# germannp/yalla

Hardware: AMD Instinct MI355X
Metric: cell-updates/sec at 1M cells (Grid_solver) (higher is better)
Workload: dtype f32

## Files before the change

include/solvers.cuh:

```cuda
#pragma once

#include <hip/hip_runtime.h>
#include <hip/hip_ext.h>

#include <assert.h>
#include <math.h>
#include <stdio.h>
#include <stdlib.h>
#include <string.h>

#include <functional>
#include <mutex>
#include <type_traits>
#include <utility>
#include <vector>

#include "cudebug.cuh"
#include "dtypes.cuh"
#include "fold256.cuh"
#include "yalla_hip.h"

#ifndef YALLA_NO_THRUST
#include <thrust/execution_policy.h>
#include <thrust/fill.h>
// ... 1543 lines not shown
        return float3{f.src[0], f.src[1], f.src[2]};
    else if constexpr (S == Fix_src::partials)
        return fixed_velocity_from_partials<N_floats<Pt>::value>(f.src, f.arg, n);
    else
        return fix_from_total(f.src, N_floats<Pt>::value, f.arg);
}
template<typename Pt>
__device__ __forceinline__ Pt minus_fix(Pt dX, const float3 fix)
{
    dX.x -= fix.x;
    dX.y -= fix.y;
    dX.z -= fix.z;
    return dX;
}
template<typename Pt>
__device__ __forceinline__ Pt heun_row(const int i, const float dt, const float* __restrict__ d_fix, const float3 fix1,
    Pt* __restrict__ d_dX, const Pt* __restrict__ d_dX1, Pt* __restrict__ d_X, float3* __restrict__ d_old_v,
    const bool zero_dX)
{
    const Pt dX_raw = d_dX[i];
    if (zero_dX) d_dX[i] = ya::zero<Pt>();
    const Pt dX = minus_fix(dX_raw, float3{d_fix[0], d_fix[1], d_fix[2]});
    const Pt dX1 = minus_fix(d_dX1[i], fix1);
    Pt X = d_X[i];
    X += (dX + dX1) * 0.5 * dt;
    d_X[i] = X;
    d_old_v[i] = float3{(dX.x + dX1.x) * 0.5f, (dX.y + dX1.y) * 0.5f, (dX.z + dX1.z) * 0.5f};
    return X;
}
}


template<typename Pt, ya::Fix_src S>
__global__ __launch_bounds__(ya::UPDATE_BLOCK) void euler_step(const int n, const float dt, const ya::Fix_args fix_args,
    const Pt* __restrict__ d_dX, const Pt* __restrict__ d_X0, Pt* __restrict__ d_X1, const Pt* __restrict__ d_dX_sorted,
    ya::Entry<Pt>* __restrict__ d_sorted, const int n_active, Pt* __restrict__ d_zero, float* __restrict__ pred_partial,
    const ya::Guard_band band)
{
    const float3 fix = ya::resolve_fix<S, Pt>(fix_args, n);
    const int i = blockIdx.x * ya::UPDATE_BLOCK + threadIdx.x;
    if (i == 0 && fix_args.out) {
        fix_args.out[0] = fix.x;
        fix_args.out[1] = fix.y;
        fix_args.out[2] = fix.z;
    }
    float moved = 0.f;
    if (i < n) {
        if (d_X1) {
            const Pt X0 = d_X0[i];
            const Pt X1 = X0 + ya::minus_fix(d_dX[i], fix) * dt;
            d_X1[i] = X1;
            moved = fabsf(X1.z - X0.z) * band.weight(X0.z);
        }
        if (d_sorted) {
            ya::Entry<Pt> e = d_sorted[i];
            Pt dX = d_dX_sorted[i];
            if constexpr (S == ya::Fix_src::totals)
                if (e.id >= n_active) dX = d_dX[e.id];
            const float z0 = e.X.z;
            e.X = e.X + ya::minus_fix(dX, fix) * dt;
            d_sorted[i] = e;
            moved = fabsf(e.X.z - z0) * band.weight(z0);
        }
        if (d_zero) d_zero[i] = ya::zero<Pt>();
    }
    if constexpr (S == ya::Fix_src::totals)
        if (pred_partial) ya::block_max_to(moved, pred_partial);
}

template<typename Pt, ya::Fix_src S>
__global__ __launch_bounds__(ya::UPDATE_BLOCK) void heun_step(const int n, const float dt, const float* __restrict__ d_fix,
    const ya::Fix_args fix1_args, Pt* __restrict__ d_dX, const Pt* __restrict__ d_dX1, Pt* __restrict__ d_X,
    float3* __restrict__ d_old_v, const bool zero_dX, const float* __restrict__ z_selected,
    float* __restrict__ moved_partial, const ya::Guard_band band, float* __restrict__ votes_out)
{
    const float3 fix1 = ya::resolve_fix<S, Pt>(fix1_args, n);
    const int i = blockIdx.x * ya::UPDATE_BLOCK + threadIdx.x;
    float moved = 0.f;
    if (i < n) {
        const Pt X = ya::heun_row(i, dt, d_fix, fix1, d_dX, d_dX1, d_X, d_old_v, zero_dX);
        if (z_selected) moved = fabsf(X.z - z_selected[i]) * band.weight(z_selected[i]);
    }
    if constexpr (S == ya::Fix_src::totals) {
        if (votes_out && i == 0) {
            votes_out[0] = fix1_args.src[ya::N_floats<Pt>::value + 2];
            votes_out[1] = fix1_args.src[ya::N_floats<Pt>::value + 3];
        }
        if (moved_partial) ya::block_max_to(moved, moved_partial);
    }
}


namespace ya {
template<typename T>
__global__ __launch_bounds__(UPDATE_BLOCK) void permute_rows(const int n, const int* __restrict__ order,
    const T* __restrict__ src, T* __restrict__ dst)
{
    const int s = blockIdx.x * UPDATE_BLOCK + threadIdx.x;
    if (s < n) dst[s] = src[order[s]];
}
__global__ __launch_bounds__(UPDATE_BLOCK) void invert_order(const int n, const int* __restrict__ order,
    int* __restrict__ new_id)
{
// ... 31 lines not shown
        else
            h_X = (Pt*)calloc(n_max, sizeof(Pt));
    }
    ~Solution()
    {
        if (h_X_locked)
            (void)ya_host_free(h_X);
        else
            free(h_X);
        free(h_n);
    }
    Solution(const Solution&) = delete;

private:
    bool h_X_locked = false;

public:
    void copy_to_device()
    {
        assert(*h_n <= n_max);
        YA_CHECK(ya_memcpy_h2d(d_X, h_X, (size_t)n_max * sizeof(Pt)));
        YA_CHECK(ya_memcpy_h2d(d_n, h_n, sizeof(int)));
    }
    void copy_to_host()
    {
        YA_CHECK(ya_memcpy_d2h(h_X, d_X, (size_t)n_max * sizeof(Pt)));
        YA_CHECK(ya_memcpy_d2h(h_n, d_n, sizeof(int)));
        assert(*h_n <= n_max);
        Solver<Pt>::check_status();
    }
    int get_d_n() { return Solver<Pt>::get_d_n(); }
    template<Pairwise_interaction<Pt> pw_int>
    void take_step(float dt, Generic_forces<Pt> gen_forces = no_gen_forces<Pt>)
    {
        return Solver<Pt>::template take_step<pw_int, friction_w_neighbour<Pt>>(
            dt, gen_forces);
    }
    template<Pairwise_interaction<Pt> pw_int, Pairwise_friction<Pt> pw_friction>
    void take_step(float dt, Generic_forces<Pt> gen_forces = no_gen_forces<Pt>)
    {
        return Solver<Pt>::template take_step<pw_int, pw_friction>(dt, gen_forces);
    }
    template<Pairwise_interaction<Pt> pw_int, typename Gen2,
        typename = decltype(std::declval<Gen2&>()((const Pt*)nullptr, (Pt*)nullptr))>
    void take_step(float dt, Gen2 gen_forces)
    {
        take_step<pw_int>(dt, Generic_forces<Pt>{[gen_forces](const int, const Pt* d_X,
                                                     Pt* d_dX) mutable { gen_forces(d_X, d_dX); }});
    }
    template<Pairwise_interaction<Pt> pw_int, Pairwise_friction<Pt> pw_friction, typename Gen2,
        typename = decltype(std::declval<Gen2&>()((const Pt*)nullptr, (Pt*)nullptr))>
    void take_step(float dt, Gen2 gen_forces)
    {
        take_step<pw_int, pw_friction>(dt,
            Generic_forces<Pt>{[gen_forces](const int, const Pt* d_X, Pt* d_dX) mutable {
                gen_forces(d_X, d_dX);
// ... 84 lines not shown
    }

    template<typename... Arrays>
    void keep_in_cube_order(const int every, Arrays&... arrays)
    {
        keep_order_every = every;
        keep_order_wait = 0;
        if (every > 0)
            keep_order = [this, &arrays...]() { this->renumber(arrays...); };
        else
            keep_order = nullptr;
    }

    int graph_steps = 0;
    long graph_launches = 0;

protected:
#ifndef YA_GRAPH_MAX_CELLS
#define YA_GRAPH_MAX_CELLS 400000
#endif
    struct Step_key {
        const void* functors = nullptr;
        int n = -1;
        float dt = 0, cube_size = 0;
        typename Computer<Pt>::Step_variant variant{};
        int fix_mode = 0, fix_point = 0;
        bool fold = true;
        bool operator==(const Step_key& o) const
        {
            return functors == o.functors && n == o.n && dt == o.dt && cube_size == o.cube_size &&
// ... 234 lines not shown
        if (Computer<Pt>::use_sorted_pipeline()) {
            Computer<Pt>::begin_build(d_X, d_n, n_max, n_reader);
            YA_CHECK(ya_n_read_end(n_reader, &n));
            assert(n <= n_max);
        } else {
            n = get_d_n();
        }
        if (n <= 0) {
            Computer<Pt>::cancel_build();
            return;
        }

        heun_stages<pw_int, pw_friction>(n, dt, gen_forces);
        last_key = sorted_path ? key_of<pw_int, pw_friction>(n, dt) : Step_key{};
    }
};


const auto TILE_SIZE = 32;

template<typename Pt>
class Tile_computer {
public:
    Tile_computer(int n_max) {}
    ya::Profiler profiler;
    bool use_sorted_pipeline() const { return false; }
    int lanes_per_cell = 0;

protected:
    hipStream_t stream = nullptr;
    float step_cube_size() const { return 0; }
    using Step_variant = int;
    Step_variant step_variant() const { return 0; }
    template<Pairwise_interaction<Pt> pw_int, Pairwise_friction<Pt> pw_friction>
    bool ready_to_capture(int) const { return false; }
    void check_status() {}
    void begin_build(const Pt*, const int*, int, ya_n_reader*) {}
    void cancel_build() {}
    const int* cube_order(int, const Pt*) { return nullptr; }
    void ids_changed() {}
    const Pt* sorted_rhs() const { return nullptr; }
    ya::Entry<Pt>* sorted_cells() { return nullptr; }
    template<Pairwise_interaction<Pt> pw_int, Pairwise_friction<Pt> pw_friction>
    void pwints_from_sorted(int, Pt*, int, bool) {}
    template<Pairwise_interaction<Pt> pw_int, Pairwise_friction<Pt> pw_friction>
    void pwints(const int n, const Pt* __restrict__ d_X, const float3* __restrict__ d_old_v,
        Pt* d_dX, const bool has_gen, const int n_active, const bool keep_sorted)
    {
        assert(n_active == n);
        hipEvent_t start, stop;
        profiler.next(&start, &stop);
        int lanes = lanes_per_cell;
        if (lanes == 0) lanes = ya::stateless_pair<Pt, pw_int, pw_friction>() ? (n <= 4096 ? 64 : 16) : 1;
        if (lanes >= 64)
            hipExtLaunchKernelGGL((ya::tile_force_coop<Pt, pw_int, pw_friction, 64>), dim3((n + 3) / 4),
                dim3(256), 0, stream, start, stop, 0, n, d_X, d_old_v, d_dX, has_gen);
        else if (lanes > 1)
            hipExtLaunchKernelGGL((ya::tile_force_coop<Pt, pw_int, pw_friction, 16>), dim3((n + 15) / 16),
                dim3(256), 0, stream, start, stop, 0, n, d_X, d_old_v, d_dX, has_gen);
// ... 49 lines not shown
    template<typename Pt>
    void build_sorted_begin(const Pt* d_X, const int* d_n, const int n_bound, const float cube_size, ya_n_reader* reader)
    {
        YA_CHECK(ya_grid_build_sorted_begin_publish(handle, d_X, sizeof(Pt), d_n, n_bound, cube_size, reader, nullptr));
    }
    template<typename Pt>
    void build_sorted_finish(const int n, const Pt* d_X, const float3* d_old_v,
        ya::Entry<Pt>* d_sorted, float4* d_sorted_v)
    {
        YA_CHECK(ya_grid_build_sorted_finish(handle, d_X, sizeof(Pt), d_old_v, n, d_sorted,
            sizeof(ya::Entry<Pt>), d_sorted_v, nullptr));
    }
    template<typename Pt>
    void rebuild_sorted(const int n, const ya::Entry<Pt>* d_prev, const float4* d_prev_v,
        const float cube_size, ya::Entry<Pt>* d_sorted, float4* d_sorted_v,
        hipStream_t stream = nullptr)
    {
        YA_CHECK(ya_grid_rebuild_sorted(handle, d_prev, sizeof(ya::Entry<Pt>), sizeof(Pt),
            d_prev_v, n, cube_size, d_sorted, d_sorted_v, stream));
    }
    const int* offsets() const { return d_offs; }
    void forget_order() { YA_CHECK(ya_grid_forget_order(handle)); }
    void set_cube_range(const int cube_lo, const int cube_hi) { YA_CHECK(ya_grid_set_cube_range(handle, cube_lo, cube_hi)); }
    void check_status()
    {
        int bits = 0;
        YA_CHECK(ya_grid_status(handle, &bits, 1));
        if (bits & YA_STATUS_OUT_OF_RANGE) {
            fprintf(stderr,
                "yalla-hip: a cell left the cube range its z-slab promised the grid (Grid::set_cube_range): it "
                "moved more than a cube between two selections of the mirrored cells.\n");
            abort();
        }
        if (bits & YA_STATUS_SCAN_STALLED) {
// ... 48 lines not shown
                        (x - 1) + shift[y] * grid_size + shift[z] * grid_size * grid_size;
        YA_CHECK((int)hipMemcpyToSymbol(HIP_SYMBOL(d_nhood), h_nhood, sizeof(h_nhood)));
        YA_CHECK(ya_malloc((void**)&d_sorted, (size_t)n_max * sizeof(ya::Entry<Pt>)));
        YA_CHECK(ya_malloc((void**)&d_sorted_v, (size_t)n_max * sizeof(float4)));
        YA_CHECK(ya_malloc((void**)&d_resorted, (size_t)n_max * sizeof(ya::Entry<Pt>)));
        YA_CHECK(ya_malloc((void**)&d_resorted_v, (size_t)n_max * sizeof(float4)));
        YA_CHECK(ya_malloc((void**)&d_dX_sorted, (size_t)n_max * sizeof(Pt)));
    }
    ~Grid_computer()
    {
        ya_free(d_sorted);
        ya_free(d_sorted_v);
        ya_free(d_resorted);
        ya_free(d_resorted_v);
        ya_free(d_dX_sorted);
        for (int p = 0; p < 3; p++) ya_free(d_tail_exchange[p]), ya_free(d_tail_tickets[p]);
        if (interior_stream && interior_stream_owned) (void)hipStreamDestroy(interior_stream);
        if (grid_built) {
            (void)hipEventDestroy(grid_built);
            (void)hipEventDestroy(interior_done);
        }
    }
    Grid_computer(const Grid_computer&) = delete;
    int force_tail_tiles = -1;
    float* d_tail_exchange[3] = {nullptr, nullptr, nullptr};
    int* d_tail_tickets[3] = {nullptr, nullptr, nullptr};
    int tail_room[3] = {0, 0, 0};
    template<auto Kernel>
    static int resident_workgroups()
    {
// ... 256 lines not shown
            grid.build_sorted_finish(n, d_X, d_old_v, d_sorted, d_sorted_v);
        else
            grid.build_sorted(n, d_X, d_old_v, cube_size, d_sorted, d_sorted_v, stream);
        build_begun = false;
        forces<pw_int, pw_friction>(n, d_sorted, d_sorted_v, d_dX, has_gen, n_active,
            keep_sorted ? d_dX_sorted : nullptr);
    }
    const Pt* sorted_rhs() const { return d_dX_sorted; }
    ya::Entry<Pt>* sorted_cells() { return d_sorted; }
    template<Pairwise_interaction<Pt> pw_int, Pairwise_friction<Pt> pw_friction>
    void pwints_from_sorted(const int n, Pt* d_dX, const int n_active, const bool has_gen)
    {
        grid.rebuild_sorted(n, d_sorted, d_sorted_v, cube_size, d_resorted, d_resorted_v, stream);
        forces<pw_int, pw_friction>(n, d_resorted, d_resorted_v, d_dX, has_gen, n_active, nullptr);
    }
};

template<typename Pt>
using Grid_solver = Heun_solver<Pt, Grid_computer>;


template<typename Pt>
class Gabriel_computer : public Grid_computer<Pt> {
public:
    float gabriel_coefficient;
    Gabriel_computer(
        int n_max, int grid_size = 50, float cube_size = 1, float gabriel_coefficient = 0.8)
        : Grid_computer<Pt>{n_max, grid_size, cube_size}, gabriel_coefficient{gabriel_coefficient}
    {
        YA_CHECK(ya_malloc((void**)&d_dense, (size_t)(n_max + 2) * sizeof(int)));
    }
    ~Gabriel_computer()
    {
        ya_free(d_dense);
        if (d_workspace) ya_free(d_workspace);
    }
    Gabriel_computer(const Gabriel_computer&) = delete;
    bool use_sorted_pipeline() const { return false; }

protected:
    int* d_dense = nullptr;
    float* d_workspace = nullptr;
    size_t workspace_floats = 0;
    template<Pairwise_interaction<Pt> pw_int, Pairwise_friction<Pt> pw_friction>
    void pwints(const int n, const Pt* __restrict__ d_X, const float3* __restrict__ d_old_v,
        Pt* d_dX, const bool has_gen, const int n_active, const bool keep_sorted)
    {
        assert(n_active == n);
        this->grid.build_sorted(n, d_X, d_old_v, this->cube_size, this->d_sorted, this->d_sorted_v);
        if (this->force_variant == 0) {
#ifdef YA_EXPERIMENTAL_FORCE_VARIANTS
            ya::gabriel_force_direct<Pt, pw_int, pw_friction><<<(n + 63) / 64, 64>>>(n, this->d_sorted,
                this->d_sorted_v, this->grid.d_cube_id, this->grid.offsets(), this->grid.grid_size,
// ... 33 lines not shown
```

include/yalla_hip.h:

```cpp
#ifndef YALLA_HIP_H
#define YALLA_HIP_H

#include <stddef.h>

#ifdef __cplusplus
extern "C" {
#endif
#pragma GCC visibility push(default)

#define YA_ABI_VERSION 10

#define YA_STATUS_OUT_OF_GRID 1

#define YA_STATUS_OUT_OF_RANGE 2

#define YA_STATUS_SCAN_STALLED 4

int ya_abi_version(void);

int ya_malloc(void** d_ptr, size_t bytes);
int ya_free(void* d_ptr);
int ya_memset_async(void* d_ptr, int value, size_t bytes, void* stream);
int ya_memcpy_h2d(void* d_dst, const void* h_src, size_t bytes);
int ya_memcpy_d2h(void* h_dst, const void* d_src, size_t bytes);
// ... 30 lines not shown
int ya_grid_build_sorted(ya_grid* g, const void* d_X, size_t stride_bytes,
    const void* d_old_v, int n, float cube_size, void* d_sorted_X,
    size_t entry_bytes, void* d_sorted_v, void* stream);

int ya_grid_build_sorted_begin(ya_grid* g, const void* d_X, size_t stride_bytes, const int* d_n,
    int n_bound, float cube_size, void* stream);
int ya_grid_build_sorted_finish(ya_grid* g, const void* d_X, size_t stride_bytes,
    const void* d_old_v, int n, void* d_sorted_X, size_t entry_bytes, void* d_sorted_v,
    void* stream);
int ya_grid_build_sorted_begin_publish(ya_grid* g, const void* d_X, size_t stride_bytes, const int* d_n,
    int n_bound, float cube_size, ya_n_reader* reader, void* stream);

int ya_grid_rebuild_sorted(ya_grid* g, const void* d_prev_sorted, size_t entry_bytes,
    size_t point_bytes, const void* d_prev_sorted_v, int n, float cube_size, void* d_sorted_out,
    void* d_sorted_v_out, void* stream);

int ya_grid_forget_order(ya_grid* g);

int ya_grid_set_cube_range(ya_grid* g, int cube_lo, int cube_hi);

int ya_grid_status(ya_grid* g, int* bits, int clear);


int ya_reduce_mean(const void* d_v, int n_floats, int n, float* d_out,
    float* d_workspace, void* stream);

int ya_reduce_sum_packed(const void* d_v, int n_floats, int n, float* d_out, float* d_workspace,
    void* stream);

int ya_reduce_partials(const void* d_v, int n_floats, int n, float* d_workspace, int* n_partials, void* stream);
// ... 72 lines not shown
```

yalla_amd/_ffi.py:

```python
import ctypes as C
import functools
import os

_HERE = os.path.dirname(os.path.abspath(__file__))
DEVICE_LIB = os.environ.get("YALLA_MODELS_LIB") or os.path.join(_HERE, "libyalla_models.so")
DEVICE_LIB_FAST = os.path.join(_HERE, "libyalla_models_fast.so")
CORE_LIB = os.path.join(_HERE, "libyalla_hip.so")
ENSEMBLE_LIB = os.path.join(_HERE, "libyalla_ensemble.so")
GRID_ENSEMBLE_LIB = os.path.join(_HERE, "libyalla_ensemble_grid.so")
GABRIEL_ENSEMBLE_LIB = os.path.join(_HERE, "libyalla_ensemble_gabriel.so")
LINKED_ENSEMBLE_LIB = os.path.join(_HERE, "libyalla_ensemble_links.so")

_pf = C.POINTER(C.c_float)
_pi = C.POINTER(C.c_int)
_sim = C.c_void_p

MODELS_ABI = {
    "ya_models_is_device": (C.c_int, []),
    "ya_models_arith": (C.c_int, []),
    "ya_models_count": (C.c_int, []),
    "ya_models_name": (C.c_char_p, [C.c_int]),
    "ya_sim_create": (C.c_int, [C.c_char_p, C.c_int, C.c_int, C.c_float, C.POINTER(_sim)]),
    "ya_sim_destroy": (None, [_sim]),
    "ya_sim_n_floats": (C.c_int, [_sim]),
# ... 69 lines not shown
GABRIEL_ENSEMBLE_ABI["ya_gabens_dense_cells"] = (C.c_int, [_ens])

LINKED_ENSEMBLE_ABI = {name.replace("ya_ens_", "ya_lens_"): sig for name, sig in ENSEMBLE_ABI.items()}
LINKED_ENSEMBLE_ABI["ya_lens_create"] = (C.c_int, [C.c_char_p, C.c_int, C.c_int, C.c_int, C.c_float, C.POINTER(_ens)])
LINKED_ENSEMBLE_ABI["ya_lens_h_link"] = (_pi, [_ens])
LINKED_ENSEMBLE_ABI["ya_lens_set_n_links"] = (C.c_int, [_ens, C.c_int])
LINKED_ENSEMBLE_ABI["ya_lens_get_n_links"] = (C.c_int, [_ens])
LINKED_ENSEMBLE_ABI["ya_lens_whole_step_lanes_used"] = (C.c_int, [_ens])
LINKED_ENSEMBLE_ABI["ya_lens_lds_bytes"] = (C.c_long, [C.c_char_p, C.c_int, C.c_int, C.c_int])

CORE_ABI = [
    "ya_abi_version", "ya_malloc", "ya_free", "ya_memset_async", "ya_memcpy_h2d",
    "ya_memcpy_d2h", "ya_host_alloc", "ya_host_free", "ya_memcpy_d2d_async", "ya_device_synchronize", "ya_get_n",
    "ya_grid_create", "ya_grid_destroy", "ya_grid_arrays", "ya_grid_offsets",
    "ya_grid_build", "ya_grid_build_sorted", "ya_grid_build_sorted_begin", "ya_grid_build_sorted_begin_publish",
    "ya_grid_build_sorted_finish", "ya_grid_rebuild_sorted", "ya_n_reader_create", "ya_n_reader_destroy",
    "ya_n_read_begin", "ya_n_read_end", "ya_grid_status", "ya_reduce_mean", "ya_reduce_sum_packed",
    "ya_reduce_workspace_bytes", "ya_select_z", "ya_select_workspace_bytes", "ya_gather_rows",
    "ya_gather_rows_pair",
    "ya_append_rows", "ya_comm_unique_id", "ya_comm_create", "ya_comm_create_loopback", "ya_comm_create_from_env",
    "ya_comm_destroy", "ya_comm_rank", "ya_comm_world", "ya_comm_exchange", "ya_comm_exchange_v",
    "ya_comm_allreduce_sum", "ya_comm_allreduce_host", "ya_comm_self_exchange", "ya_comm_info", "ya_reduce_partials",
    "ya_shader_clock_mhz", "ya_grid_set_cube_range", "ya_grid_forget_order", "ya_copy_component", "ya_pack_cells", "ya_append_cells", "ya_fill_holes", "ya_find_id", "ya_max_abs_diff", "ya_max_abs_diff_partials",
    "ya_slab_guard_update", "ya_slab_pack", "ya_async_read_create", "ya_async_read_destroy",
    "ya_async_read_begin", "ya_async_read_end", "ya_async_read_target", "ya_async_read_mark",
]


def _load(path, table):
    if not os.path.exists(path):
        raise FileNotFoundError(
# ... 47 lines not shown
```

yalla_amd/csrc/core.hip:

```cpp
#include <hip/hip_runtime.h>
#include <stdio.h>
#include <stdlib.h>
#include <string.h>

#include <mutex>
#include <unordered_map>

#include "cube_id.cuh"
#include "fold256.cuh"
#include "yalla_hip.h"

namespace {
using ya::cube_id_of;
using ya::fold256;

constexpr int BLOCK = 256;
constexpr int SCAN_ITEMS = 8;
constexpr int SCAN_TILE = BLOCK * SCAN_ITEMS;
constexpr int REDUCE_MAX_BLOCKS = 1024;

inline int ceil_div(long a, long b) { return (int)((a + b - 1) / b); }


__device__ __forceinline__ int visit(int s, const int* __restrict__ prev_pid, int n_prev, int n)
// ... 195 lines not shown
        for (int k = 0; k < NW; k++) v[k] = src[k];
#pragma unroll
        for (int k = 0; k < NW; k++) out[k] = v[k];
        out[NW] = __int_as_float(p);
        const float* ov = old_v + (size_t)p * 3;
        sorted_v[dst] = make_float4(ov[0], ov[1], ov[2], 0.f);
    }
}

template<int EW>
__global__ __launch_bounds__(BLOCK) void k_order_from(const int* __restrict__ arrival_pid,
    const int* __restrict__ arrival_src, const int* __restrict__ cube_id_sorted,
    const int* __restrict__ offs, int n,
    const unsigned* __restrict__ prev_entries, const float4* __restrict__ prev_v,
    int* __restrict__ point_id, int* __restrict__ next_prev_pid, unsigned* __restrict__ sorted_out,
    float4* __restrict__ sorted_v_out)
{
    int s = blockIdx.x * BLOCK + threadIdx.x;
    if (s >= n) return;
    const int c = cube_id_sorted[s];
    const int a = offs[c], b = offs[c + 1];
    const int src = arrival_src[s];
    const unsigned* mine = prev_entries + (size_t)src * EW;
    const int p = arrival_pid[s];
    int smaller = 0;
    for (int t = a; t < b; t++) smaller += arrival_pid[t] < p;
    const int dst = a + smaller;
    point_id[dst] = p;
    next_prev_pid[dst] = p;
    unsigned w[EW];
#pragma unroll
    for (int k = 0; k < EW; k++) w[k] = mine[k];
    unsigned* out = sorted_out + (size_t)dst * EW;
#pragma unroll
    for (int k = 0; k < EW; k++) out[k] = w[k];
    sorted_v_out[dst] = prev_v[src];
}

static_assert(BLOCK == 256, "the reduction kernels fold with ya::fold256");

template<int NW>
__global__ __launch_bounds__(BLOCK) void k_reduce_partial(
    const float* __restrict__ v, int n, float* __restrict__ partials)
{
    __shared__ float sh[NW * BLOCK];
    float acc[NW];
#pragma unroll
    for (int k = 0; k < NW; k++) acc[k] = 0.f;
    for (long i = (long)blockIdx.x * BLOCK + threadIdx.x; i < n; i += (long)gridDim.x * BLOCK) {
        const float* p = v + (size_t)i * NW;
#pragma unroll
// ... 738 lines not shown

int ya_grid_build_sorted_finish(ya_grid* g, const void* d_X, size_t stride_bytes,
    const void* d_old_v, int n, void* d_sorted_X, size_t entry_bytes, void* d_sorted_v, void* stream)
{
    if (!d_sorted_X ||
        !sorted_args_ok(g, n, stride_bytes, d_old_v, d_sorted_X, entry_bytes, d_sorted_v))
        return (int)hipErrorInvalidValue;
    return build_finish(
        g, d_X, stride_bytes, d_old_v, n, d_sorted_X, entry_bytes, d_sorted_v, (hipStream_t)stream);
}

int ya_grid_rebuild_sorted(ya_grid* g, const void* d_prev_sorted, size_t entry_bytes,
    size_t point_bytes, const void* d_prev_sorted_v, int n, float cube_size, void* d_sorted_out,
    void* d_sorted_v_out, void* stream)
{
    if (!g || n < 0 || n > g->n_max || point_bytes < 12 || entry_bytes < point_bytes + 4 ||
        entry_bytes % 4 || point_bytes % 4 || !d_prev_sorted || !d_prev_sorted_v || !d_sorted_out ||
        !d_sorted_v_out)
        return (int)hipErrorInvalidValue;
    hipStream_t st = (hipStream_t)stream;
    const int entry_f = (int)(entry_bytes / 4);
    const int nb = ceil_div(n, BLOCK);
    if (n > 0)
        k_bin<<<nb, BLOCK, 0, st>>>((const float*)d_prev_sorted, entry_f, n, cube_size, g->grid_size,
            g->n_cubes, g->d_prev_pid, 0, g->d_cube_of, g->d_rank, g->d_count, g->d_status,
            nullptr, 0, nullptr, g->range_lo, g->range_hi);
    launch_scan(g, n, nullptr, st);
    if (n > 0) {
        const int id_word = (int)(point_bytes / 4);
        k_scatter<<<nb, BLOCK, 0, st>>>(g->d_cube_of, g->d_rank, g->d_offs, n, g->d_prev_pid, 0,
            g->d_arrival, g->d_cube_id, g->d_arrival_src, (const unsigned*)d_prev_sorted, entry_f,
            id_word, nullptr);
#define YA_ORDER_FROM(EW)                                                                    \
    case EW:                                                                                 \
        k_order_from<EW><<<nb, BLOCK, 0, st>>>(g->d_arrival, g->d_arrival_src, g->d_cube_id, \
            g->d_offs, n, (const unsigned*)d_prev_sorted, (const float4*)d_prev_sorted_v,    \
            g->d_point_id, g->d_prev_pid, (unsigned*)d_sorted_out, (float4*)d_sorted_v_out); \
        break;
        switch (entry_f) {
            YA_ORDER_FROM(4)
            YA_ORDER_FROM(5)
            YA_ORDER_FROM(6)
            YA_ORDER_FROM(7)
            YA_ORDER_FROM(8)
            YA_ORDER_FROM(9)
            YA_ORDER_FROM(10)
            YA_ORDER_FROM(11)
            YA_ORDER_FROM(12)
            YA_ORDER_FROM(13)
            YA_ORDER_FROM(14)
            YA_ORDER_FROM(15)
            YA_ORDER_FROM(16)
// ... 446 lines not shown
```

yalla_amd/csrc/models_harness.inc:

```

#include <math.h>

#include <memory>
#include <string>
#include <vector>

#include "yalla_models.h"

#ifdef YA_ORACLE
#include "gabriel_host.h"
#endif

namespace harness {

struct Sim_base {
    virtual ~Sim_base() {}
    virtual int n_floats() = 0;
    virtual int n_max() = 0;
    virtual float* h_X() = 0;
    virtual int* h_n() = 0;
    virtual void copy_to_device() = 0;
    virtual void copy_to_host() = 0;
    virtual int get_d_n() = 0;
    virtual void take_steps(float dt, int n_steps) = 0;
    virtual void set_fixed(int mode, int point) = 0;
    virtual int set_cube_size(float) { return -2; }
    virtual void random_sphere(float dist_to_nb, unsigned seed) = 0;
    virtual void get_old_v(float* out) = 0;
    virtual void set_old_v(const float* in) = 0;
    virtual int get_grid(int*, int*, int*, int*) { return -2; }
    virtual int build_grid(int gs, float cs, int*, int*, int*, int*) = 0;
    virtual int set_param(const char*, double) { return -2; }
    virtual int set_prop(const char*, const int*, int) { return -2; }
    virtual int get_prop(const char*, int*, int) { return -2; }
    virtual int set_links(const int*, int, float) { return -2; }
    virtual int set_reduce_order(int) { return -1; }
    virtual int profile(int) { return -1; }
    virtual int profile_read(double*, int*) { return -1; }
    virtual long graph_launches() { return -1; }
    virtual int slab_init(float, float, float, const int*) { return -2; }
    virtual int slab_decompose(const float*, int, int, int, float) { return -2; }
    virtual int slab_n_own() { return -2; }
    virtual int slab_n_local() { return -2; }
    virtual int slab_get_own(float*, int*) { return -2; }
    virtual int slab_setup(int, int, int, int) { return -2; }
    virtual int slab_set_transport(ya_slab_exchange_fn, ya_slab_allreduce_fn, void*) { return -2; }
    virtual int slab_use_rccl(void*) { return -2; }
    virtual int slab_step(float, int) { return -2; }
    virtual long slab_info(int) { return -2; }
};

template<typename Pt>
using Harness_slab_solver = Slab_grid_solver_impl<Pt, harness_ops>;

// ... 206 lines not shown
    if (cube_id) YA_D2H(cube_id, g.d_cube_id, (size_t)n_max * sizeof(int));
    if (point_id) YA_D2H(point_id, g.d_point_id, (size_t)n_max * sizeof(int));
    if (cube_start) YA_D2H(cube_start, g.d_cube_start, (size_t)g.n_cubes * sizeof(int));
    if (cube_end) YA_D2H(cube_end, g.d_cube_end, (size_t)g.n_cubes * sizeof(int));
    return 0;
}

template<typename Pt>
struct No_gen {
    template<typename C>
    Generic_forces<Pt> gen(C&) { return no_gen_forces<Pt>; }
    template<typename C>
    void pre_step(C&) {}
    template<typename C>
    void post_step(C&, float) {}
    template<typename C>
    int keep_in_cube_order(C& cells, int every)
    {
        cells.keep_in_cube_order(every);
        return 0;
    }
    int set_links(const int*, int, float) { return -2; }
    int set_param(const char*, double) { return -2; }
    template<typename C>
    int renumber_now(C& cells)
    {
        cells.renumber();
        return 0;
    }
    template<typename C>
// ... 141 lines not shown

inline const void*& growth_symbols_owner()
{
    static const void* owner = nullptr;
    return owner;
}

template<typename Rule, bool PROLIFERATE_FIRST>
struct Growth_policy : public No_gen<typename Rule::Pt> {
    using Pt = typename Rule::Pt;
    std::unique_ptr<Property<int>> type, mes_nbs, epi_nbs, scratch;
    float rate = 0.f;
    double mean_dist = 0.75;
    unsigned seed = 1, step = 0;
    bool reset_nbs = true;
    template<typename C>
    void ensure(C& cells)
    {
        if (type) return;
        type.reset(new Property<int>{cells.n_max});
        mes_nbs.reset(new Property<int>{cells.n_max});
        epi_nbs.reset(new Property<int>{cells.n_max});
        scratch.reset(new Property<int>{cells.n_max + cells.n_max / 1024 + 2});
        type->copy_to_device();
        mes_nbs->copy_to_device();
        epi_nbs->copy_to_device();
    }
    template<typename C>
    void bind(C& cells)
    {
// ... 102 lines not shown
    Pairwise_friction<Pt> pw_friction, typename Policy>
struct Sim : public Sim_base {
    Cells<Pt, SOLVER> cells;
    Policy policy;
    Sim(int n_max, int gs, float cs) : cells{n_max, gs, cs} {}

    int n_floats() override { return sizeof(Pt) / sizeof(float); }
    int n_max() override { return cells.n_max; }
    float* h_X() override { return reinterpret_cast<float*>(cells.h_X); }
    int* h_n() override { return cells.h_n; }
    void copy_to_device() override { cells.copy_to_device(); }
    void copy_to_host() override { cells.copy_to_host(); }
    int get_d_n() override { return cells.get_d_n(); }
    void take_steps(float dt, int n_steps) override
    {
        for (int s = 0; s < n_steps; s++) {
            policy.pre_step(cells);
            cells.template take_step<pw_int, pw_friction>(dt, policy.gen(cells));
            policy.post_step(cells, dt);
        }
    }
    void set_fixed(int mode, int point) override
    {
        if (mode == 0) cells.set_fixed();
        if (mode == 1) cells.set_fixed(point);
        if (mode == 2) cells.set_fixed_xy(point);
    }
    int set_cube_size(float cs) override { return cells.set_cube_size(cs); }
    void random_sphere(float dist_to_nb, unsigned seed) override
    {
// ... 27 lines not shown
        if (std::string(name) == "coop_lanes") return cells.set_coop_lanes((int)v);
        if (std::string(name) == "stage_v_max") return cells.set_stage_v_max((int)v);
        if (std::string(name) == "tail_tiles") return cells.set_tail_tiles((int)v);
        if (std::string(name) == "gather_offset_bits") return cells.set_gather_offset_bits((int)v);
        if (std::string(name) == "sum_order") return cells.set_sum_order((int)v);
        if (std::string(name) == "sorted_pipeline") return cells.set_sorted_pipeline((int)v);
        if (std::string(name) == "graph") return cells.set_graph((int)v);
        if (std::string(name) == "tile_lanes") return cells.set_tile_lanes((int)v);
        if (std::string(name) == "slab_global_ids") return cells.set_slab_global_ids((int)v);
        if (std::string(name) == "gabriel_coefficient") return cells.set_gabriel_coefficient((float)v);
        if (std::string(name) == "renumber_now") return policy.renumber_now(cells);
        if (std::string(name) == "renumber_every") return policy.keep_in_cube_order(cells, (int)v);
        if (std::string(name) == "slab_guard") return cells.set_slab_guard((int)v);
        if (std::string(name) == "slab_guard_lag") return cells.set_slab_guard_lag((float)v);
        if (std::string(name) == "slab_local_order") return cells.set_slab_local_order((int)v);
#ifndef YA_ORACLE
        if (std::string(name) == "links_segmented_min") {
            ya::links_segmented_min() = (int)v;
            return 0;
        }
#endif
        return policy.set_param(name, v);
    }
    int set_links(const int* ab, int n, float s) override { return policy.set_links(ab, n, s); }
    int set_prop(const char* name, const int* v, int n) override { return policy.set_prop(cells, name, v, n); }
    int get_prop(const char* name, int* v, int n) override { return policy.get_prop(cells, name, v, n); }
    int slab_init(float a, float b, float h, const int* gid) override { return cells.slab_init(a, b, h, gid, *cells.h_n); }
    int slab_decompose(const float* X, int n, int rank, int world, float cube_size) override
    {
        const Pt* whole = reinterpret_cast<const Pt*>(X);
// ... 22 lines not shown
    }
    int slab_step(float dt, int migrate) override
    {
        const int rc = cells.template slab_step<pw_int, pw_friction>(dt, migrate, policy.gen(cells));
        if (rc == 0) *cells.h_n = cells.slab.n_own;
        return rc;
    }
    long graph_launches() override
    {
#ifdef YA_ORACLE
        return -1;
#else
        return cells.graph_launches_so_far();
#endif
    }
#ifdef YA_ORACLE
    int set_reduce_order(int order) override
    {
        cells.reduce_order = order ? YA_REDUCE_TREE : YA_REDUCE_SERIAL;
        return 0;
    }
#else
    int profile(int enable) override
    {
        cells.profiler.enable(enable != 0, enable);
        return 0;
    }
    int profile_read(double* ms, int* launches) override
    {
        cells.profiler.read(ms, launches);
// ... 216 lines not shown
#ifdef YA_ORACLE
    return -1;
#else
    unsigned long long* d_bad = (unsigned long long*)harness_ops::alloc(8);
    YA_ZERO(d_bad, 8);
    ya::check_reciprocal_all<<<4096, 256>>>(first_bits, last_bits, d_bad);
    unsigned long long bad = 0;
    YA_D2H(&bad, d_bad, 8);
    harness_ops::release(d_bad);
    return (long)bad;
#endif
}
int ya_sim_profile(ya_sim* s, int enable) { return s->p->profile(enable); }
int ya_sim_profile_read(ya_sim* s, double* ms, int* launches) { return s->p->profile_read(ms, launches); }
long ya_sim_graph_launches(ya_sim* s) { return s->p->graph_launches(); }

}
```

yalla_amd/solution.py:

```python
import ctypes as C

import numpy as np

from . import _ffi


class YallaError(RuntimeError):
    pass


def _check(code, what):
    if code != 0:
        raise YallaError(f"{what} failed with harness code {code}")


def _ip(a):
    return a.ctypes.data_as(C.POINTER(C.c_int))


class Solution:
    def __init__(self, model, n_max, grid_size=50, cube_size=1.0, lib=None):
        self.lib = lib if lib is not None else _ffi.device_lib()
        self.model = model
        self.grid_size = int(grid_size)
# ... 112 lines not shown
    def get_prop(self, name, n):
        v = np.empty(int(n), dtype=np.int32)
        _check(self.lib.ya_sim_get_prop(self._h, name.encode(), _ip(v), len(v)), "get_prop")
        return v

    def set_links(self, pairs, strength=0.2):
        ab = np.ascontiguousarray(pairs, dtype=np.int32).reshape(-1, 2)
        _check(self.lib.ya_sim_set_links(self._h, _ip(ab), len(ab), float(strength)), "set_links")

    def set_reduce_order(self, order):
        return self.lib.ya_sim_set_reduce_order(self._h, int(order))

    def graph_launches(self):
        return self.lib.ya_sim_graph_launches(self._h)

    def profile(self, enable, every=1):
        return self.lib.ya_sim_profile(self._h, int(every) if enable else 0)

    def profile_read(self):
        ms = C.c_double()
        launches = C.c_int()
        _check(self.lib.ya_sim_profile_read(self._h, C.byref(ms), C.byref(launches)),
               "profile_read")
        return ms.value, launches.value


def models(lib=None):
    lib = lib if lib is not None else _ffi.device_lib()
    return [lib.ya_models_name(i).decode() for i in range(lib.ya_models_count())]
```

Measured before the change: 868.8 million.

## Carry sorted cell order across multi-step batches instead of rebuilding from scratch

Adds a take_steps path that keeps the cells in cube-sorted order across consecutive Heun steps. Each stage reorders from the previous sorted array with a slot map, so the full grid build and the scatter back to id order are skipped on intermediate steps. A new heun_step_sorted kernel updates entries in sorted order and writes back to d_X/d_old_v only on the last step. This costs extra buffers and an indirect gather of dX1. It only applies when there are no generic forces, no graph capture, the COM is fixed and the order is not kept.

```diff
diff --git a/include/solvers.cuh b/include/solvers.cuh
--- a/include/solvers.cuh
+++ b/include/solvers.cuh
@@ -1581,18 +1581,24 @@
     return dX;
 }
 template<typename Pt>
+__device__ __forceinline__ float3 heun_update(Pt& X, const Pt dX_raw, const Pt dX1_raw, const float3 fix,
+    const float3 fix1, const float dt)
+{
+    const Pt dX = minus_fix(dX_raw, fix);
+    const Pt dX1 = minus_fix(dX1_raw, fix1);
+    X += (dX + dX1) * 0.5 * dt;
+    return float3{(dX.x + dX1.x) * 0.5f, (dX.y + dX1.y) * 0.5f, (dX.z + dX1.z) * 0.5f};
+}
+template<typename Pt>
 __device__ __forceinline__ Pt heun_row(const int i, const float dt, const float* __restrict__ d_fix, const float3 fix1,
     Pt* __restrict__ d_dX, const Pt* __restrict__ d_dX1, Pt* __restrict__ d_X, float3* __restrict__ d_old_v,
     const bool zero_dX)
 {
     const Pt dX_raw = d_dX[i];
     if (zero_dX) d_dX[i] = ya::zero<Pt>();
-    const Pt dX = minus_fix(dX_raw, float3{d_fix[0], d_fix[1], d_fix[2]});
-    const Pt dX1 = minus_fix(d_dX1[i], fix1);
     Pt X = d_X[i];
-    X += (dX + dX1) * 0.5 * dt;
+    d_old_v[i] = heun_update(X, dX_raw, d_dX1[i], float3{d_fix[0], d_fix[1], d_fix[2]}, fix1, dt);
     d_X[i] = X;
-    d_old_v[i] = float3{(dX.x + dX1.x) * 0.5f, (dX.y + dX1.y) * 0.5f, (dX.z + dX1.z) * 0.5f};
     return X;
 }
 }
@@ -1602,7 +1608,7 @@
 __global__ __launch_bounds__(ya::UPDATE_BLOCK) void euler_step(const int n, const float dt, const ya::Fix_args fix_args,
     const Pt* __restrict__ d_dX, const Pt* __restrict__ d_X0, Pt* __restrict__ d_X1, const Pt* __restrict__ d_dX_sorted,
     ya::Entry<Pt>* __restrict__ d_sorted, const int n_active, Pt* __restrict__ d_zero, float* __restrict__ pred_partial,
-    const ya::Guard_band band)
+    const ya::Guard_band band, ya::Entry<Pt>* __restrict__ d_sorted_out = nullptr)
 {
     const float3 fix = ya::resolve_fix<S, Pt>(fix_args, n);
     const int i = blockIdx.x * ya::UPDATE_BLOCK + threadIdx.x;
@@ -1626,7 +1632,7 @@
                 if (e.id >= n_active) dX = d_dX[e.id];
             const float z0 = e.X.z;
             e.X = e.X + ya::minus_fix(dX, fix) * dt;
-            d_sorted[i] = e;
+            (d_sorted_out ? d_sorted_out : d_sorted)[i] = e;
             moved = fabsf(e.X.z - z0) * band.weight(z0);
         }
         if (d_zero) d_zero[i] = ya::zero<Pt>();
@@ -1654,6 +1660,26 @@
             votes_out[1] = fix1_args.src[ya::N_floats<Pt>::value + 3];
         }
         if (moved_partial) ya::block_max_to(moved, moved_partial);
+    }
+}
+
+template<typename Pt>
+__global__ __launch_bounds__(ya::UPDATE_BLOCK) void heun_step_sorted(const int n, const float dt,
+    const float* __restrict__ d_fix, const ya::Fix_args fix1_args, const ya::Entry<Pt>* __restrict__ d_sorted,
+    const Pt* __restrict__ d_dX_sorted, const int* __restrict__ d_slot2, const Pt* __restrict__ d_dX1_sorted,
+    ya::Entry<Pt>* __restrict__ d_out, float4* __restrict__ d_out_v, Pt* __restrict__ d_X, float3* __restrict__ d_old_v)
+{
+    const float3 fix1 = ya::resolve_fix<ya::Fix_src::partials, Pt>(fix1_args, n);
+    const int s = blockIdx.x * ya::UPDATE_BLOCK + threadIdx.x;
+    if (s >= n) return;
+    ya::Entry<Pt> e = d_sorted[s];
+    const float3 v = ya::heun_update(e.X, d_dX_sorted[s], d_dX1_sorted[d_slot2[s]],
+        float3{d_fix[0], d_fix[1], d_fix[2]}, fix1, dt);
+    d_out[s] = e;
+    d_out_v[s] = make_float4(v.x, v.y, v.z, 0.f);
+    if (d_X) {
+        d_X[e.id] = e.X;
+        d_old_v[e.id] = v;
     }
 }
 
@@ -1715,6 +1741,16 @@
 
 private:
     bool h_X_locked = false;
+    template<typename S>
+    static auto decomposed(const S& solver, int) -> decltype((bool)solver.slab.on)
+    {
+        return solver.slab.on;
+    }
+    template<typename S>
+    static bool decomposed(const S&, long)
+    {
+        return false;
+    }
 
 public:
     void copy_to_device()
@@ -1741,6 +1777,17 @@
     void take_step(float dt, Generic_forces<Pt> gen_forces = no_gen_forces<Pt>)
     {
         return Solver<Pt>::template take_step<pw_int, pw_friction>(dt, gen_forces);
+    }
+    template<Pairwise_interaction<Pt> pw_int>
+    void take_steps(float dt, int k, Generic_forces<Pt> gen_forces = no_gen_forces<Pt>)
+    {
+        take_steps<pw_int, friction_w_neighbour<Pt>>(dt, k, gen_forces);
+    }
+    template<Pairwise_interaction<Pt> pw_int, Pairwise_friction<Pt> pw_friction>
+    void take_steps(float dt, int k, Generic_forces<Pt> gen_forces = no_gen_forces<Pt>)
+    {
+        if (!decomposed(*this, 0)) return Solver<Pt>::template take_steps<pw_int, pw_friction>(dt, k, gen_forces);
+        for (int s = 0; s < k; s++) Solver<Pt>::template take_step<pw_int, pw_friction>(dt, gen_forces);
     }
     template<Pairwise_interaction<Pt> pw_int, typename Gen2,
         typename = decltype(std::declval<Gen2&>()((const Pt*)nullptr, (Pt*)nullptr))>
@@ -1855,6 +1902,8 @@
 
     int graph_steps = 0;
     long graph_launches = 0;
+    bool carry_sorted = true;
+    long carried_steps = 0;
 
 protected:
 #ifndef YA_GRAPH_MAX_CELLS
@@ -2119,6 +2168,54 @@
         heun_stages<pw_int, pw_friction>(n, dt, gen_forces);
         last_key = sorted_path ? key_of<pw_int, pw_friction>(n, dt) : Step_key{};
     }
+
+    template<Pairwise_interaction<Pt> pw_int, Pairwise_friction<Pt> pw_friction>
+    void take_steps(const float dt, const int k, Generic_forces<Pt> gen_forces)
+    {
+        if (take_steps_carried<pw_int, pw_friction>(dt, k, gen_forces)) return;
+        for (int s = 0; s < k; s++) take_step<pw_int, pw_friction>(dt, gen_forces);
+    }
+    template<Pairwise_interaction<Pt> pw_int, Pairwise_friction<Pt> pw_friction>
+    bool take_steps_carried(const float dt, const int k, Generic_forces<Pt>& gen_forces)
+    {
+        if (!carry_sorted || k < 2 || graph_steps != 0 || keep_order) return false;
+        if (!(fix_com and !fix_com_z and fold_in_update) || !ya::is_no_gen_forces<Pt>(gen_forces)) return false;
+        if (!Computer<Pt>::carry_ready(n_max)) return false;
+        int n;
+        Computer<Pt>::begin_build(d_X, d_n, n_max, n_reader);
+        YA_CHECK(ya_n_read_end(n_reader, &n));
+        assert(n <= n_max);
+        if (n <= 0) {
+            Computer<Pt>::cancel_build();
+            for (int s = 1; s < k; s++) take_step<pw_int, pw_friction>(dt, gen_forces);
+            return true;
+        }
+        const int blocks = (n + ya::UPDATE_BLOCK - 1) / ya::UPDATE_BLOCK;
+        for (int s = 0; s < k; s++) {
+            int n_partials = 0;
+            if (s == 0)
+                Computer<Pt>::template pwints<pw_int, pw_friction>(n, d_X, d_old_v, d_dX, false, n, true);
+            else
+                Computer<Pt>::template pwints_carried<pw_int, pw_friction>(1, n, d_dX);
+            YA_CHECK(ya_reduce_partials(d_dX, n_floats, n, d_workspace, &n_partials, this->stream));
+            euler_step<Pt, Fix::partials><<<blocks, ya::UPDATE_BLOCK, 0, this->stream>>>(n, dt,
+                ya::Fix_args{d_workspace, n_partials, d_mean_first}, d_dX, d_X, nullptr, Computer<Pt>::sorted_rhs(),
+                Computer<Pt>::sorted_cells(), n, nullptr, nullptr, ya::Guard_band{}, Computer<Pt>::carried_cells());
+            Computer<Pt>::template pwints_carried<pw_int, pw_friction>(2, n, d_dX1);
+            YA_CHECK(ya_reduce_partials(d_dX1, n_floats, n, d_workspace, &n_partials, this->stream));
+            const bool last = s == k - 1;
+            heun_step_sorted<Pt><<<blocks, ya::UPDATE_BLOCK, 0, this->stream>>>(n, dt, d_mean_first,
+                ya::Fix_args{d_workspace, n_partials}, Computer<Pt>::sorted_cells(), Computer<Pt>::sorted_rhs(),
+                Computer<Pt>::carried_slots(), Computer<Pt>::carried_rhs(), Computer<Pt>::carried_cells(),
+                Computer<Pt>::carried_v(), last ? d_X : nullptr, last ? d_old_v : nullptr);
+        }
+        stage1_fix = d_mean_first;
+        sorted_stage_cells = -1;
+        rhs_zeroed[0] = rhs_zeroed[1] = 0;
+        last_key = key_of<pw_int, pw_friction>(n, dt);
+        carried_steps += k - 1;
+        return true;
+    }
 };
 
 
@@ -2148,6 +2245,13 @@
     ya::Entry<Pt>* sorted_cells() { return nullptr; }
     template<Pairwise_interaction<Pt> pw_int, Pairwise_friction<Pt> pw_friction>
     void pwints_from_sorted(int, Pt*, int, bool) {}
+    bool carry_ready(int) { return false; }
+    template<Pairwise_interaction<Pt> pw_int, Pairwise_friction<Pt> pw_friction>
+    void pwints_carried(int, int, Pt*) {}
+    ya::Entry<Pt>* carried_cells() { return nullptr; }
+    float4* carried_v() { return nullptr; }
+    const Pt* carried_rhs() const { return nullptr; }
+    const int* carried_slots() const { return nullptr; }
     template<Pairwise_interaction<Pt> pw_int, Pairwise_friction<Pt> pw_friction>
     void pwints(const int n, const Pt* __restrict__ d_X, const float3* __restrict__ d_old_v,
         Pt* d_dX, const bool has_gen, const int n_active, const bool keep_sorted)
@@ -2227,10 +2331,10 @@
     template<typename Pt>
     void rebuild_sorted(const int n, const ya::Entry<Pt>* d_prev, const float4* d_prev_v,
         const float cube_size, ya::Entry<Pt>* d_sorted, float4* d_sorted_v,
-        hipStream_t stream = nullptr)
-    {
-        YA_CHECK(ya_grid_rebuild_sorted(handle, d_prev, sizeof(ya::Entry<Pt>), sizeof(Pt),
-            d_prev_v, n, cube_size, d_sorted, d_sorted_v, stream));
+        hipStream_t stream = nullptr, int* d_slot_of_prev = nullptr)
+    {
+        YA_CHECK(ya_grid_rebuild_sorted_map(handle, d_prev, sizeof(ya::Entry<Pt>), sizeof(Pt),
+            d_prev_v, n, cube_size, d_sorted, d_sorted_v, d_slot_of_prev, stream));
     }
     const int* offsets() const { return d_offs; }
     void forget_order() { YA_CHECK(ya_grid_forget_order(handle)); }
@@ -2309,6 +2413,7 @@
         ya_free(d_resorted);
         ya_free(d_resorted_v);
         ya_free(d_dX_sorted);
+        if (d_carried) ya_free(d_carried), ya_free(d_carried_rhs), ya_free(d_carried_slots);
         for (int p = 0; p < 3; p++) ya_free(d_tail_exchange[p]), ya_free(d_tail_tickets[p]);
         if (interior_stream && interior_stream_owned) (void)hipStreamDestroy(interior_stream);
         if (grid_built) {
@@ -2595,6 +2700,42 @@
         grid.rebuild_sorted(n, d_sorted, d_sorted_v, cube_size, d_resorted, d_resorted_v, stream);
         forces<pw_int, pw_friction>(n, d_resorted, d_resorted_v, d_dX, has_gen, n_active, nullptr);
     }
+    ya::Entry<Pt>* d_carried = nullptr;
+    Pt* d_carried_rhs = nullptr;
+    int* d_carried_slots = nullptr;
+    bool carry_ready(const int n_max)
+    {
+        if (!use_sorted_pipeline() || d_global_id || force_part != 0) return false;
+        if (d_carried) return true;
+        if (carry_refused) return false;
+        const int rc[3] = {ya_malloc((void**)&d_carried, (size_t)n_max * sizeof(ya::Entry<Pt>)),
+            ya_malloc((void**)&d_carried_rhs, (size_t)n_max * sizeof(Pt)),
+            ya_malloc((void**)&d_carried_slots, (size_t)n_max * sizeof(int))};
+        if (rc[0] == 0 && rc[1] == 0 && rc[2] == 0) return true;
+        if (rc[0] == 0) ya_free(d_carried);
+        if (rc[1] == 0) ya_free(d_carried_rhs);
+        if (rc[2] == 0) ya_free(d_carried_slots);
+        d_carried = nullptr, d_carried_rhs = nullptr, d_carried_slots = nullptr;
+        (void)hipGetLastError();
+        carry_refused = true;
+        return false;
+    }
+    bool carry_refused = false;
+    template<Pairwise_interaction<Pt> pw_int, Pairwise_friction<Pt> pw_friction>
+    void pwints_carried(const int stage, const int n, Pt* d_dX)
+    {
+        if (stage == 1) {
+            grid.rebuild_sorted(n, d_carried, d_resorted_v, cube_size, d_sorted, d_sorted_v, stream);
+            forces<pw_int, pw_friction>(n, d_sorted, d_sorted_v, d_dX, false, n, d_dX_sorted);
+        } else {
+            grid.rebuild_sorted(n, d_carried, d_sorted_v, cube_size, d_resorted, d_resorted_v, stream, d_carried_slots);
+            forces<pw_int, pw_friction>(n, d_resorted, d_resorted_v, d_dX, false, n, d_carried_rhs);
+        }
+    }
+    ya::Entry<Pt>* carried_cells() { return d_carried; }
+    float4* carried_v() { return d_resorted_v; }
+    const Pt* carried_rhs() const { return d_carried_rhs; }
+    const int* carried_slots() const { return d_carried_slots; }
 };
 
 template<typename Pt>
@@ -2618,6 +2759,7 @@
     }
     Gabriel_computer(const Gabriel_computer&) = delete;
     bool use_sorted_pipeline() const { return false; }
+    bool carry_ready(int) { return false; }
 
 protected:
     int* d_dense = nullptr;
diff --git a/include/yalla_hip.h b/include/yalla_hip.h
--- a/include/yalla_hip.h
+++ b/include/yalla_hip.h
@@ -68,6 +68,9 @@
 int ya_grid_rebuild_sorted(ya_grid* g, const void* d_prev_sorted, size_t entry_bytes,
     size_t point_bytes, const void* d_prev_sorted_v, int n, float cube_size, void* d_sorted_out,
     void* d_sorted_v_out, void* stream);
+int ya_grid_rebuild_sorted_map(ya_grid* g, const void* d_prev_sorted, size_t entry_bytes,
+    size_t point_bytes, const void* d_prev_sorted_v, int n, float cube_size, void* d_sorted_out,
+    void* d_sorted_v_out, int* d_slot_of_prev, void* stream);
 
 int ya_grid_forget_order(ya_grid* g);
 
diff --git a/yalla_amd/_ffi.py b/yalla_amd/_ffi.py
--- a/yalla_amd/_ffi.py
+++ b/yalla_amd/_ffi.py
@@ -107,7 +107,7 @@
     "ya_memcpy_d2h", "ya_host_alloc", "ya_host_free", "ya_memcpy_d2d_async", "ya_device_synchronize", "ya_get_n",
     "ya_grid_create", "ya_grid_destroy", "ya_grid_arrays", "ya_grid_offsets",
     "ya_grid_build", "ya_grid_build_sorted", "ya_grid_build_sorted_begin", "ya_grid_build_sorted_begin_publish",
-    "ya_grid_build_sorted_finish", "ya_grid_rebuild_sorted", "ya_n_reader_create", "ya_n_reader_destroy",
+    "ya_grid_build_sorted_finish", "ya_grid_rebuild_sorted", "ya_grid_rebuild_sorted_map", "ya_n_reader_create", "ya_n_reader_destroy",
     "ya_n_read_begin", "ya_n_read_end", "ya_grid_status", "ya_reduce_mean", "ya_reduce_sum_packed",
     "ya_reduce_workspace_bytes", "ya_select_z", "ya_select_workspace_bytes", "ya_gather_rows",
     "ya_gather_rows_pair",
diff --git a/yalla_amd/csrc/core.hip b/yalla_amd/csrc/core.hip
--- a/yalla_amd/csrc/core.hip
+++ b/yalla_amd/csrc/core.hip
@@ -233,7 +233,7 @@
     const int* __restrict__ offs, int n,
     const unsigned* __restrict__ prev_entries, const float4* __restrict__ prev_v,
     int* __restrict__ point_id, int* __restrict__ next_prev_pid, unsigned* __restrict__ sorted_out,
-    float4* __restrict__ sorted_v_out)
+    float4* __restrict__ sorted_v_out, int* __restrict__ slot_of_src)
 {
     int s = blockIdx.x * BLOCK + threadIdx.x;
     if (s >= n) return;
@@ -254,6 +254,7 @@
 #pragma unroll
     for (int k = 0; k < EW; k++) out[k] = w[k];
     sorted_v_out[dst] = prev_v[src];
+    if (slot_of_src) slot_of_src[src] = dst;
 }
 
 static_assert(BLOCK == 256, "the reduction kernels fold with ya::fold256");
@@ -1022,6 +1023,14 @@
     size_t point_bytes, const void* d_prev_sorted_v, int n, float cube_size, void* d_sorted_out,
     void* d_sorted_v_out, void* stream)
 {
+    return ya_grid_rebuild_sorted_map(g, d_prev_sorted, entry_bytes, point_bytes, d_prev_sorted_v, n, cube_size,
+        d_sorted_out, d_sorted_v_out, nullptr, stream);
+}
+
+int ya_grid_rebuild_sorted_map(ya_grid* g, const void* d_prev_sorted, size_t entry_bytes,
+    size_t point_bytes, const void* d_prev_sorted_v, int n, float cube_size, void* d_sorted_out,
+    void* d_sorted_v_out, int* d_slot_of_prev, void* stream)
+{
     if (!g || n < 0 || n > g->n_max || point_bytes < 12 || entry_bytes < point_bytes + 4 ||
         entry_bytes % 4 || point_bytes % 4 || !d_prev_sorted || !d_prev_sorted_v || !d_sorted_out ||
         !d_sorted_v_out)
@@ -1043,7 +1052,8 @@
     case EW:                                                                                 \
         k_order_from<EW><<<nb, BLOCK, 0, st>>>(g->d_arrival, g->d_arrival_src, g->d_cube_id, \
             g->d_offs, n, (const unsigned*)d_prev_sorted, (const float4*)d_prev_sorted_v,    \
-            g->d_point_id, g->d_prev_pid, (unsigned*)d_sorted_out, (float4*)d_sorted_v_out); \
+            g->d_point_id, g->d_prev_pid, (unsigned*)d_sorted_out, (float4*)d_sorted_v_out,  \
+            d_slot_of_prev);                                                                 \
         break;
         switch (entry_f) {
             YA_ORDER_FROM(4)
diff --git a/yalla_amd/csrc/models_harness.inc b/yalla_amd/csrc/models_harness.inc
--- a/yalla_amd/csrc/models_harness.inc
+++ b/yalla_amd/csrc/models_harness.inc
@@ -38,6 +38,9 @@
     virtual int profile(int) { return -1; }
     virtual int profile_read(double*, int*) { return -1; }
     virtual long graph_launches() { return -1; }
+#if YA_IS_DEVICE
+    virtual long carried_steps() = 0;
+#endif
     virtual int slab_init(float, float, float, const int*) { return -2; }
     virtual int slab_decompose(const float*, int, int, int, float) { return -2; }
     virtual int slab_n_own() { return -2; }
@@ -274,6 +277,9 @@
     void pre_step(C&) {}
     template<typename C>
     void post_step(C&, float) {}
+#if YA_IS_DEVICE
+    static constexpr bool steps_alone = true;
+#endif
     template<typename C>
     int keep_in_cube_order(C& cells, int every)
     {
@@ -445,6 +451,9 @@
     double mean_dist = 0.75;
     unsigned seed = 1, step = 0;
     bool reset_nbs = true;
+#if YA_IS_DEVICE
+    static constexpr bool steps_alone = false;
+#endif
     template<typename C>
     void ensure(C& cells)
     {
@@ -577,6 +586,15 @@
     int get_d_n() override { return cells.get_d_n(); }
     void take_steps(float dt, int n_steps) override
     {
+#if YA_IS_DEVICE
+        if (Policy::steps_alone) {
+            Generic_forces<Pt> gen = policy.gen(cells);
+            if (ya::is_no_gen_forces<Pt>(gen)) {
+                cells.template take_steps<pw_int, pw_friction>(dt, n_steps, gen);
+                return;
+            }
+        }
+#endif
         for (int s = 0; s < n_steps; s++) {
             policy.pre_step(cells);
             cells.template take_step<pw_int, pw_friction>(dt, policy.gen(cells));
@@ -634,6 +652,12 @@
         if (std::string(name) == "slab_guard") return cells.set_slab_guard((int)v);
         if (std::string(name) == "slab_guard_lag") return cells.set_slab_guard_lag((float)v);
         if (std::string(name) == "slab_local_order") return cells.set_slab_local_order((int)v);
+#if YA_IS_DEVICE
+        if (std::string(name) == "carry_sorted") {
+            cells.carry_sorted = v != 0;
+            return 0;
+        }
+#endif
 #ifndef YA_ORACLE
         if (std::string(name) == "links_segmented_min") {
             ya::links_segmented_min() = (int)v;
@@ -686,6 +710,9 @@
         return cells.graph_launches_so_far();
 #endif
     }
+#if YA_IS_DEVICE
+    long carried_steps() override { return cells.carried_steps; }
+#endif
 #ifdef YA_ORACLE
     int set_reduce_order(int order) override
     {
@@ -932,5 +959,8 @@
 int ya_sim_profile(ya_sim* s, int enable) { return s->p->profile(enable); }
 int ya_sim_profile_read(ya_sim* s, double* ms, int* launches) { return s->p->profile_read(ms, launches); }
 long ya_sim_graph_launches(ya_sim* s) { return s->p->graph_launches(); }
-
-}
+#if YA_IS_DEVICE
+__attribute__((visibility("default"))) long ya_sim_carried_steps(ya_sim* s) { return s->p->carried_steps(); }
+#endif
+
+}
diff --git a/yalla_amd/solution.py b/yalla_amd/solution.py
--- a/yalla_amd/solution.py
+++ b/yalla_amd/solution.py
@@ -150,6 +150,13 @@
     def graph_launches(self):
         return self.lib.ya_sim_graph_launches(self._h)
 
+    def carried_steps(self):
+        fn = getattr(self.lib, "ya_sim_carried_steps", None)
+        if fn is None:
+            return -1
+        fn.restype, fn.argtypes = C.c_long, [C.c_void_p]
+        return fn(self._h)
+
     def profile(self, enable, every=1):
         return self.lib.ya_sim_profile(self._h, int(every) if enable else 0)
 
```

After: 882.3 million, median of 6. +1.6%, better.
